# lelecaruso/NavierStokes_Project_NM4PDE

Measured on AMD Instinct MI355X. Metric: time-steps/sec (assemble_time_step + solve_time_step), 3D flow past a cylinder, P2/P1, Yosida, per-rank ILU(0), higher is better.
Workload: dtype f64

## Files before the change

navierstokes_project_nm4pde_amd/csrc/nsx_cg.hip:

```cpp
#include "nsx_grid.hpp"

namespace nsx {

constexpr int CG_THREADS = 256;
constexpr int CG_NW = CG_THREADS / 64, CG_NG = CG_THREADS / 16;
constexpr int CG_MAXB = 256;
constexpr int CG_MAX_WG = 1024;
constexpr int CG_NV = 3;
constexpr int CG_RING = 4;
constexpr size_t CG_REGION = (size_t)CG_RING * CG_NV * CG_MAX_WG + (size_t)CG_RING * CG_NV;
enum { S_CGP = 100 };

__device__ __forceinline__ double ld_agent(const double *p) { return __hip_atomic_load(p, __ATOMIC_RELAXED, __HIP_MEMORY_SCOPE_AGENT); }
__device__ __forceinline__ void st_agent(double *p, double v) { __hip_atomic_store(p, v, __ATOMIC_RELAXED, __HIP_MEMORY_SCOPE_AGENT); }

template <int W>
__device__ __forceinline__ double cg_group_sum(double v) {
  v += dpp_f64<0xB1>(v);
  v += dpp_f64<0x4E>(v);
  if (W >= 8) v += dpp_f64<0x141>(v);
  if (W >= 16) v += dpp_f64<0x140>(v);
  return v;
}

struct CgBox {
  unsigned long long *row, *row2, *total, *total2;
};
__device__ __forceinline__ CgBox cg_box_of(unsigned long long *box, int e) {
  CgBox b;
  b.row = box + (size_t)(e % CG_RING) * CG_NV * CG_MAX_WG;
  b.row2 = box + (size_t)((e + 2) % CG_RING) * CG_NV * CG_MAX_WG;
  b.total = box + (size_t)CG_RING * CG_NV * CG_MAX_WG + (size_t)(e % CG_RING) * CG_NV;
  b.total2 = box + (size_t)CG_RING * CG_NV * CG_MAX_WG + (size_t)((e + 2) % CG_RING) * CG_NV;
  return b;
}
__device__ __forceinline__ double cg_sum8(const double *w) {
  if (CG_NW == 4) return (w[0] + w[1]) + (w[2] + w[3]);
  return ((w[0] + w[1]) + (w[2] + w[3])) + ((w[4] + w[5]) + (w[6] + w[7]));
}

template <int NV>
__device__ __forceinline__ void cg_post(const double (&part)[NV], unsigned long long *box, int e, int nwg, double (*sh)[CG_NV * 8], int *s_err, bool drop = false) {
  const int wg = blockIdx.x, tid = threadIdx.x, wave = tid >> 6;
  const CgBox bx = cg_box_of(box, e);
  double *buf = sh[2 * (e & 1)], *buf0 = sh[2 * (e & 1) + 1];
  double ws[NV];
#pragma unroll
  for (int v = 0; v < NV; ++v) ws[v] = gx_wave_sum(part[v]);
  asm volatile("s_waitcnt vmcnt(0)" ::: "memory");
  if ((tid & 63) == 0) {
#pragma unroll
    for (int v = 0; v < NV; ++v) buf[v * 8 + wave] = ws[v];
  }
  __syncthreads();
  if (tid == 0) {
#pragma unroll
    for (int v = 0; v < NV; ++v)
      if (!drop) gx_post(bx.row + (size_t)v * CG_MAX_WG + wg, cg_sum8(buf + v * 8));
#pragma unroll
    for (int v = 0; v < CG_NV; ++v) gx_clear(bx.row2 + (size_t)v * CG_MAX_WG + wg);
  }
  if (wg == 0) {
    int lerr = 0;
    double a[NV];
#pragma unroll
    for (int v = 0; v < NV; ++v) a[v] = 0.0;
    for (int q = tid; q < nwg; q += CG_THREADS) {
      double m[NV];
      gx_wait_n<NV>(bx.row + q, CG_MAX_WG, m, &lerr);
#pragma unroll
      for (int v = 0; v < NV; ++v) a[v] += m[v];
    }
    if (lerr) *s_err = 1;
#pragma unroll
    for (int v = 0; v < NV; ++v) ws[v] = gx_wave_sum(a[v]);
    if ((tid & 63) == 0) {
#pragma unroll
      for (int v = 0; v < NV; ++v) buf0[v * 8 + wave] = ws[v];
    }
    __syncthreads();
    if (tid == 0 && !*s_err) {
#pragma unroll
      for (int v = 0; v < NV; ++v) gx_post(bx.total + v, cg_sum8(buf0 + v * 8));
    }
    if (tid < CG_NV) gx_clear(bx.total2 + tid);
  }
}
template <int NV>
__device__ __forceinline__ bool cg_collect(double (&tot)[NV], unsigned long long *box, int e, double *bc, int *s_err) {
  if (threadIdx.x == 0) {
    int lerr = 0;
    double m[NV];
    gx_wait_n<NV>(cg_box_of(box, e).total, 1, m, &lerr);
#pragma unroll
    for (int v = 0; v < NV; ++v) bc[v] = m[v];
    if (lerr) *s_err = 1;
  }
  __syncthreads();
#pragma unroll
  for (int v = 0; v < NV; ++v) tot[v] = bc[v];
  return *s_err == 0;
}
constexpr int CG_PF = 8;
constexpr int CG_MAX_UCOLS = 1024;
constexpr int CG_LPOOL = 6656;

__global__ void k_cg_pack(int64_t n_slots, const int32_t *__restrict__ src, const double *__restrict__ sv, double *__restrict__ out) {
  const int64_t i = (int64_t)blockIdx.x * blockDim.x + threadIdx.x;
  if (i < n_slots) out[i] = src[i] >= 0 ? sv[src[i]] : 0.0;
}

#define NSX_CG_LOAD(V, L, S0)                                   \
  _Pragma("unroll") for (int k = 0; k < CG_PF; ++k) {           \
    const int s_ = (S0) + k;                                    \
    const bool ok_ = s_ < s1;                                   \
    V[k] = ok_ ? sval[(size_t)s_ * 256 + tid] : 0.0;            \
    L[k] = ok_ ? (int)slidx[(size_t)s_ * 256 + tid] : 0;        \
  }
__device__ __forceinline__ void cg_spmv_prefetch(int s0, int s1, const double *__restrict__ sval, const uint16_t *__restrict__ slidx, int tid,
                                                 double (&va)[CG_PF], int (&la)[CG_PF]) {
  NSX_CG_LOAD(va, la, s0)
}
__device__ __forceinline__ void cg_block_spmv(int s0, int s1, const double *__restrict__ sval, const uint16_t *__restrict__ slidx,
                                              const int32_t *__restrict__ sinfo, const double *xst, double *hvs, int tid ,
                                              double (&va)[CG_PF], int (&la)[CG_PF]) {
  const int grp = tid >> 4, lane = tid & 15;
  double vb[CG_PF];
  int lb[CG_PF];
  double acc = 0.0;
#define NSX_CG_USE(V, L, S0)                                    \
  _Pragma("unroll") for (int k = 0; k < CG_PF; ++k) {           \
    const int s_ = (S0) + k;                                    \
    if (s_ < s1) {                                              \
      acc += V[k] * xst[L[k]];                                  \
      const int inf = sinfo[s_];                                \
      if (inf & 0x8000) {                                       \
        const double r_ = cg_group_sum<16>(acc);                \
        if (lane == 0) hvs[(inf & 0x7fff) * 16 + grp] = r_;     \
        acc = 0.0;                                              \
      }                                                         \
    }                                                           \
  }
  for (int sb = s0; sb < s1; sb += 2 * CG_PF) {
    NSX_CG_LOAD(vb, lb, sb + CG_PF)
    NSX_CG_USE(va, la, sb)
    NSX_CG_LOAD(va, la, sb + 2 * CG_PF)
    NSX_CG_USE(vb, lb, sb + CG_PF)
  }
#undef NSX_CG_USE
}
#undef NSX_CG_LOAD

template <int RPG, bool LRES>
__global__ __launch_bounds__(CG_THREADS) void k_cg_schur(const int32_t *__restrict__ bptr, const int32_t *__restrict__ u_ptr,
                                                  const int32_t *__restrict__ u_cols, const int32_t *__restrict__ s_ptr,
                                                  const double *__restrict__ sval, const uint16_t *__restrict__ slidx,
                                                  const int32_t *__restrict__ sinfo, const int64_t *__restrict__ dn_off,
                                                  const double *__restrict__ P, const double *__restrict__ b, double *x, double *D0, double *D1,
                                                  double *H, double rtol, int maxiter, unsigned long long *box, unsigned long long *box_other,
                                                  double *pub_vals, unsigned long long *pub_flag, unsigned long long seq, int *err_dev, int drop_wg,
                                                  const int32_t *__restrict__ a_rowptr, const double *__restrict__ a_val,
                                                  const uint16_t *__restrict__ a_lidx) {
  static_assert(!LRES || RPG > 0, "the LDS-resident operator needs the register-resident block inverses");
  constexpr int MAXB = RPG > 0 ? 16 * RPG : CG_MAXB;
  __shared__ double gs[MAXB], hs[MAXB], ds[MAXB], hvs[MAXB], xs[MAXB], xst[CG_MAX_UCOLS];
  __shared__ double sh[4][CG_NV * 8], bc[CG_NV];
  __shared__ int s_err;
  __shared__ double lval[LRES ? CG_LPOOL : 1];
  __shared__ uint16_t lidx[LRES ? CG_LPOOL : 2];
  __shared__ int lrow[LRES ? MAXB + 1 : 1];
  const int wg = blockIdx.x, tid = threadIdx.x, nwg = gridDim.x;
  if (tid == 0) s_err = 0;
  for (size_t q = (size_t)wg * CG_THREADS + tid; q < CG_REGION; q += (size_t)nwg * CG_THREADS) box_other[q] = GX_EMPTY;
  const int r0 = bptr[wg], nb = bptr[wg + 1] - r0;
  const int u0 = u_ptr[wg], nu = u_ptr[wg + 1] - u0;
  const int half = tid >> 8, ht = tid & 255;
  const int s0 = s_ptr[3 * wg + half], s1 = s_ptr[3 * wg + (CG_THREADS == 512 ? half + 1 : 2)];
  const double *Pb = P + dn_off[wg];
  const int grp = tid >> 4, lane = tid & 15;
  const bool own = tid < nb;
  int e = 0;
  constexpr int NU = CG_MAX_UCOLS / CG_THREADS;
  int ucol[NU];
#pragma unroll
  for (int k = 0; k < NU; ++k) ucol[k] = tid + CG_THREADS * k < nu ? u_cols[u0 + tid + CG_THREADS * k] : -1;
  if (tid < MAXB) gs[tid] = 0.0;

  double pa[8], pb[8];
  auto fetch = [&](int q, double(&pv)[8]) {
    const bool live = q < nb;
    const double *prow = Pb + (size_t)(live ? q : 0) * nb;
#pragma unroll
    for (int c = 0; c < 8; ++c) {
      const int j = lane + 16 * c;
      pv[c] = (live && j < nb) ? prow[j] : 0.0;
    }
  };
  constexpr bool PRES = RPG > 0;
  double pr[PRES ? RPG : 1][PRES ? RPG : 1];
  if constexpr (PRES) {
#pragma unroll
    for (int r = 0; r < RPG; ++r) {
      const int q = grp + CG_NG * r;
      const double *prow = Pb + (size_t)(q < nb ? q : 0) * nb;
#pragma unroll
      for (int c = 0; c < RPG; ++c) {
        const int j = lane + 16 * c;
        pr[r][c] = (q < nb && j < nb) ? prow[j] : 0.0;
      }
    }
  }
  auto prefetch_P = [&]() {
    if constexpr (!PRES) {
      if (nb <= 128) {
        fetch(grp, pa);
        fetch(grp + CG_NG, pb);
      }
    }
  };
  auto apply_P = [&]() {
    if constexpr (PRES) {
#pragma unroll
      for (int r = 0; r < RPG; ++r) {
        const int q = grp + CG_NG * r;
        if (q < nb) {
          double acc = 0.0;
#pragma unroll
          for (int c = 0; c < RPG; ++c) acc += pr[r][c] * gs[lane + 16 * c];
          acc = cg_group_sum<16>(acc);
          if (lane == 0) hs[q] = acc;
        }
      }
    } else if (nb <= 128) {
      auto use = [&](int q, const double(&pv)[8]) {
        if (q >= nb) return;
        double acc = 0.0;
#pragma unroll
        for (int c = 0; c < 8; ++c) acc += pv[c] * gs[lane + 16 * c];
        acc = cg_group_sum<16>(acc);
        if (lane == 0) hs[q] = acc;
      };
      for (int q = grp; q < nb; q += 2 * CG_NG) {
        use(q, pa);
        fetch(q + 2 * CG_NG, pa);
        use(q + CG_NG, pb);
        fetch(q + 3 * CG_NG, pb);
      }
    } else {
      for (int q = grp; q < nb; q += CG_NG) {
        const double *prow = Pb + (size_t)q * nb;
        double pv[16];
#pragma unroll
        for (int c = 0; c < 16; ++c) {
          const int j = lane + 16 * c;
          pv[c] = j < nb ? prow[j] : 0.0;
        }
        double acc = 0.0;
#pragma unroll
        for (int c = 0; c < 16; ++c) acc += pv[c] * gs[lane + 16 * c];
        acc = cg_group_sum<16>(acc);
        if (lane == 0) hs[q] = acc;
      }
    }
    __syncthreads();
    if (own) st_agent(H + r0 + tid, hs[tid]);
  };

  double va[LRES ? 1 : CG_PF];
  int la[LRES ? 1 : CG_PF];
  if constexpr (LRES) {
    const int p0 = a_rowptr[r0], nz = a_rowptr[r0 + nb] - p0;
    for (int q = tid; q < nz; q += CG_THREADS) {
      lval[q] = a_val[p0 + q];
      lidx[q] = a_lidx[p0 + q];
    }
    if (tid <= nb) lrow[tid] = a_rowptr[r0 + tid] - p0;
  }
  auto prefetch_A = [&]() {
    if constexpr (!LRES) cg_spmv_prefetch(s0, s1, sval, slidx, ht, va, la);
  };
  auto block_spmv = [&]() {
    if constexpr (LRES) {
#pragma unroll
      for (int r = 0; r < RPG; ++r) {
        const int q = grp + CG_NG * r;
        if (q < nb) {
          const int e1 = lrow[q + 1];
          double acc = 0.0;
          for (int e = lrow[q] + lane; e < e1; e += 16) acc += lval[e] * xst[lidx[e]];
          acc = cg_group_sum<16>(acc);
          if (lane == 0) hvs[q] = acc;
        }
      }
    } else {
      cg_block_spmv(s0, s1, sval, slidx, sinfo, xst, hvs, ht, va, la);
    }
  };

  double bi = 0.0;
  if (own) {
    xs[tid] = x[r0 + tid];
    bi = b[r0 + tid];
  }
#pragma unroll
  for (int k = 0; k < NU; ++k)
    if (ucol[k] >= 0) xst[tid + CG_THREADS * k] = x[ucol[k]];
  prefetch_A();
  __syncthreads();
  block_spmv();
  __syncthreads();
  prefetch_P();
  if (own) gs[tid] = hvs[tid] - bi;
  __syncthreads();
  apply_P();
  double tot3[3];
  {
    const double part[3] = {own ? gs[tid] * gs[tid] : 0.0, own ? bi * bi : 0.0, own ? gs[tid] * hs[tid] : 0.0};
    cg_post<3>(part, box, e, nwg, sh, &s_err, wg == drop_wg);
    prefetch_A();
    if (!cg_collect<3>(tot3, box, e++, bc, &s_err)) {
      if (tid == 0) __hip_atomic_store(err_dev, 1, __ATOMIC_RELAXED, __HIP_MEMORY_SCOPE_AGENT);
      if (wg == 0 && tid == 0) {
        __hip_atomic_store(pub_vals + 2, 3.0, __ATOMIC_RELAXED, __HIP_MEMORY_SCOPE_SYSTEM);
        asm volatile("s_waitcnt vmcnt(0)" ::: "memory");
        __hip_atomic_store(pub_flag, seq, __ATOMIC_RELAXED, __HIP_MEMORY_SCOPE_SYSTEM);
      }
      return;
    }
  }
  const double tol = rtol * sqrt(tot3[1]);
  double res = sqrt(tot3[0]), gh = tot3[2], beta = 0.0;
  int it = 0;
  int conv = res <= tol ? 1 : ((it >= maxiter || res != res) ? 2 : 0);
  bool dead = false;
  while (conv == 0) {
    ++it;
    const double *Dp = (it & 1) ? D0 : D1;
    double *Dc = (it & 1) ? D1 : D0;
#pragma unroll
    for (int k = 0; k < NU; ++k)
      if (ucol[k] >= 0) {
        const int j = ucol[k];
        xst[tid + CG_THREADS * k] = it == 1 ? -ld_agent(H + j) : __builtin_fma(beta, ld_agent(Dp + j), -ld_agent(H + j));
      }
    if (own) {
      const double dcur = it == 1 ? -hs[tid] : __builtin_fma(beta, ds[tid], -hs[tid]);
      ds[tid] = dcur;
      st_agent(Dc + r0 + tid, dcur);
    }
    __syncthreads();
    block_spmv();
    __syncthreads();
    double tot1[1];
    {
      const double part[1] = {own ? ds[tid] * hvs[tid] : 0.0};
      cg_post<1>(part, box, e, nwg, sh, &s_err);
      prefetch_P();
      if (!cg_collect<1>(tot1, box, e++, bc, &s_err)) {
        dead = true;
        break;
      }
    }
    const double alpha = gh / tot1[0];
    if (own) {
      xs[tid] += alpha * ds[tid];
      gs[tid] = gs[tid] + alpha * hvs[tid];
    }
    __syncthreads();
    apply_P();
    double tot2[2];
    {
      const double part[2] = {own ? gs[tid] * gs[tid] : 0.0, own ? gs[tid] * hs[tid] : 0.0};
      cg_post<2>(part, box, e, nwg, sh, &s_err);
      prefetch_A();
      if (!cg_collect<2>(tot2, box, e++, bc, &s_err)) {
        dead = true;
        break;
      }
    }
    res = sqrt(fabs(tot2[0]));
    conv = res <= tol ? 1 : ((it >= maxiter || res != res) ? 2 : 0);
    beta = tot2[1] / gh;
    gh = tot2[1];
  }
  if (dead && tid == 0) __hip_atomic_store(err_dev, 1, __ATOMIC_RELAXED, __HIP_MEMORY_SCOPE_AGENT);
  if (!dead && own) x[r0 + tid] = xs[tid];
  if (wg == 0 && tid == 0) {
    __hip_atomic_store(pub_vals + 0, (double)it, __ATOMIC_RELAXED, __HIP_MEMORY_SCOPE_SYSTEM);
    __hip_atomic_store(pub_vals + 1, res, __ATOMIC_RELAXED, __HIP_MEMORY_SCOPE_SYSTEM);
    __hip_atomic_store(pub_vals + 2, dead ? 3.0 : (conv == 1 ? 0.0 : 1.0), __ATOMIC_RELAXED, __HIP_MEMORY_SCOPE_SYSTEM);
    __hip_atomic_store(pub_vals + 3, tol, __ATOMIC_RELAXED, __HIP_MEMORY_SCOPE_SYSTEM);
    asm volatile("s_waitcnt vmcnt(0)" ::: "memory");
    __hip_atomic_store(pub_flag, seq, __ATOMIC_RELAXED, __HIP_MEMORY_SCOPE_SYSTEM);
  }
}

void build_cg_plan(nsx_handle *h) {
  CgPlan &pl = h->cgplan;
  pl.ok = false;
  const IluSchedule &s = h->schedS;
  if (!s.dense || s.max_rows > CG_MAXB) return;
  const Csr &g = h->gS.host;
  const std::vector<int32_t> &bptr = s.block_ptr_h;
  const int nb = s.n_blocks;
  std::vector<int32_t> u_ptr(nb + 1, 0), u_cols, s_ptr(3 * (size_t)nb + 1, 0), s_info, s_src, tmp;
  std::vector<uint16_t> s_lidx, a_lidx((size_t)g.nnz());
  pl.max_block_nnz = 0;
  for (int b = 0; b < nb; ++b) {
    const int r0 = bptr[b], r1 = bptr[b + 1], n = r1 - r0;
    tmp.assign(g.colind.begin() + g.rowptr[r0], g.colind.begin() + g.rowptr[r1]);
    std::sort(tmp.begin(), tmp.end());
    tmp.erase(std::unique(tmp.begin(), tmp.end()), tmp.end());
    if ((int)tmp.size() > CG_MAX_UCOLS) return;
    u_cols.insert(u_cols.end(), tmp.begin(), tmp.end());
    u_ptr[b + 1] = (int32_t)u_cols.size();
    pl.max_block_nnz = std::max(pl.max_block_nnz, g.rowptr[r1] - g.rowptr[r0]);
    for (int p = g.rowptr[r0]; p < g.rowptr[r1]; ++p) a_lidx[p] = (uint16_t)(std::lower_bound(tmp.begin(), tmp.end(), g.colind[p]) - tmp.begin());
    for (int half = 0; half < 2; ++half) {
      s_ptr[3 * (size_t)b + half] = (int32_t)s_info.size();
      for (int r = half; r * 16 < n; r += 2) {
        int maxlen = 0;
        for (int q = 16 * r; q < std::min(n, 16 * r + 16); ++q) maxlen = std::max(maxlen, g.rowptr[r0 + q + 1] - g.rowptr[r0 + q]);
        const int chunks = std::max(1, (maxlen + 15) / 16);
        for (int c = 0; c < chunks; ++c) {
          s_info.push_back(r | (c == chunks - 1 ? 0x8000 : 0));
          for (int t = 0; t < 256; ++t) {
            const int q = 16 * r + (t >> 4), e = 16 * c + (t & 15);
            int32_t src = -1;
            uint16_t li = 0;
            if (q < n && g.rowptr[r0 + q] + e < g.rowptr[r0 + q + 1]) {
              src = g.rowptr[r0 + q] + e;
              li = (uint16_t)(std::lower_bound(tmp.begin(), tmp.end(), g.colind[src]) - tmp.begin());
            }
            s_src.push_back(src);
            s_lidx.push_back(li);
          }
        }
      }
    }
    s_ptr[3 * (size_t)b + 2] = (int32_t)s_info.size();
  }
  pl.n_slots = (int64_t)s_src.size();
  pl.u_ptr.upload(u_ptr, h->stream);
  pl.u_cols.upload(u_cols, h->stream);
  pl.s_ptr.upload(s_ptr, h->stream);
  pl.s_info.upload(s_info, h->stream);
  pl.s_src.upload(s_src, h->stream);
  pl.s_lidx.upload(s_lidx, h->stream);
  pl.a_lidx.upload(a_lidx, h->stream);
  pl.s_val.alloc((size_t)pl.n_slots);
  pl.ok = true;
  pl.values_current = false;
  if (getenv("NSX_DEBUG"))
    fprintf(stderr, "[nsx] persistent Schur CG plan: %d blocks, %lld slabs (fill %.2f), unique columns per block avg %.0f\n", nb,
            (long long)s_info.size(), (double)g.nnz() / (double)std::max<int64_t>(1, pl.n_slots), (double)u_cols.size() / std::max(1, nb));
}

void cg_pack_values(nsx_handle *h) {
  CgPlan &pl = h->cgplan;
  if (!pl.ok) return;
  LaunchScope ls(h, "cg_pack", 20.0 * (double)pl.n_slots);
  hipLaunchKernelGGL(k_cg_pack, dim3(cdiv(pl.n_slots, 256)), dim3(256), 0, h->stream, pl.n_slots, pl.s_src.p, h->vSchur.p, pl.s_val.p);
  pl.values_current = true;
}

static void cg_setup(nsx_handle *h) {
  if (h->cg_box.p || h->cg_disabled) return;
  h->cg_max_wg = 0;
  if (getenv("NSX_CG_PERSISTENT") && atoi(getenv("NSX_CG_PERSISTENT")) == 0) {
    h->cg_disabled = true;
    return;
  }
  int cus = 0, per_cu = 0;
  HIP_CHECK(hipDeviceGetAttribute(&cus, hipDeviceAttributeMultiprocessorCount, h->prm.device));
  int per_cu_res[2] = {0, 0};
  HIP_CHECK(hipOccupancyMaxActiveBlocksPerMultiprocessor(&per_cu, k_cg_schur<0, false>, CG_THREADS, 0));
  HIP_CHECK(hipOccupancyMaxActiveBlocksPerMultiprocessor(&per_cu_res[0], k_cg_schur<6, false>, CG_THREADS, 0));
  HIP_CHECK(hipOccupancyMaxActiveBlocksPerMultiprocessor(&per_cu_res[1], k_cg_schur<8, false>, CG_THREADS, 0));
  h->cg_max_wg_res[0] = std::min(CG_MAX_WG, per_cu_res[0] * cus);
  h->cg_max_wg_res[1] = std::min(CG_MAX_WG, per_cu_res[1] * cus);
  int per_cu_lres[2] = {0, 0};
  HIP_CHECK(hipOccupancyMaxActiveBlocksPerMultiprocessor(&per_cu_lres[0], k_cg_schur<6, true>, CG_THREADS, 0));
  HIP_CHECK(hipOccupancyMaxActiveBlocksPerMultiprocessor(&per_cu_lres[1], k_cg_schur<8, true>, CG_THREADS, 0));
  h->cg_max_wg_lres[0] = std::min(CG_MAX_WG, per_cu_lres[0] * cus);
  h->cg_max_wg_lres[1] = std::min(CG_MAX_WG, per_cu_lres[1] * cus);
  h->cg_box.alloc(2 * CG_REGION + 2);
  HIP_CHECK(hipMemsetAsync(h->cg_box.p, 0xff, 2 * CG_REGION * sizeof(unsigned long long), h->stream));
  HIP_CHECK(hipMemsetAsync(h->cg_box.p + 2 * CG_REGION, 0, 2 * sizeof(unsigned long long), h->stream));
  h->cg_max_wg = std::min(CG_MAX_WG, per_cu * cus);
  if (getenv("NSX_DEBUG"))
    fprintf(stderr, "[nsx] persistent Schur CG: %d CUs x %d resident workgroups, grid <= %d (block inverses in registers: <= 96 rows x %d, <= 128 rows x %d; operator in LDS as well: x %d, x %d)\n", cus, per_cu,
            h->cg_max_wg, per_cu_res[0], per_cu_res[1], per_cu_lres[0], per_cu_lres[1]);
}

bool cg_schur_persistent(nsx_handle *h, double *x, const double *b, double rtol, int maxiter, int *steps, double *last, int *status) {
  const IluSchedule &s = h->schedS;
  const CgPlan &pl = h->cgplan;
  if (h->comm || !s.dense || s.max_rows > CG_MAXB || !pl.ok || !pl.values_current) return false;
  cg_setup(h);
  if (h->cg_max_wg == 0 || s.n_blocks > h->cg_max_wg) return false;
  const bool pres_ok = !(getenv("NSX_CG_PRES") && atoi(getenv("NSX_CG_PRES")) == 0);
  const int rpg = !pres_ok ? 0 : (s.max_rows <= 96 && s.n_blocks <= h->cg_max_wg_res[0]) ? 6 : (s.max_rows <= 128 && s.n_blocks <= h->cg_max_wg_res[1]) ? 8 : 0;
  const bool pres = rpg > 0;
  const bool lres_ok = !(getenv("NSX_CG_LRES") && atoi(getenv("NSX_CG_LRES")) == 0);
  const bool lres = lres_ok && pres && pl.max_block_nnz <= CG_LPOOL && s.n_blocks <= h->cg_max_wg_lres[rpg == 6 ? 0 : 1];
  const int n = h->n_p;
  if ((int)h->cg_vec.n < 3 * n) h->cg_vec.alloc((size_t)3 * n);
  double *D0 = h->cg_vec.p, *D1 = D0 + n, *H = D1 + n;
  const unsigned long long seq = ++h->pub_seq;
  unsigned long long *box = h->cg_box.p + (size_t)h->cg_parity * CG_REGION, *box_other = h->cg_box.p + (size_t)(1 - h->cg_parity) * CG_REGION;
  int *err_dev = (int *)(h->cg_box.p + 2 * CG_REGION);
  double *pub_vals = h->pub_dev + S_CGP;
  unsigned long long *pub_flag = (unsigned long long *)(h->pub_dev + N_SLOTS);
  ProfEntry *pe = nullptr;
  {
    LaunchScope ls(h, "cg_S", 0.0);
    pe = ls.e;
#define NSX_CG_GO(PRES_, LRES_)                                                                                                                       \
  hipLaunchKernelGGL((k_cg_schur<PRES_, LRES_>), dim3(s.n_blocks), dim3(CG_THREADS), 0, h->stream, s.block_ptr.p, pl.u_ptr.p, pl.u_cols.p, pl.s_ptr.p,  \
                     pl.s_val.p, pl.s_lidx.p, pl.s_info.p, s.dn_off.p, s.dn_P.p, b, x, D0, D1, H, rtol, maxiter, box, box_other, pub_vals, pub_flag, seq, \
                     err_dev, h->gx_drop_wg, h->gS.rowptr.p, h->vSchur.p, pl.a_lidx.p)
    if (rpg == 6 && lres) NSX_CG_GO(6, true); else if (rpg == 8 && lres) NSX_CG_GO(8, true);
    else if (rpg == 6) NSX_CG_GO(6, false); else if (rpg == 8) NSX_CG_GO(8, false); else NSX_CG_GO(0, false);
#undef NSX_CG_GO
    if (getenv("NSX_DEBUG") && (h->cg_resident != pres || h->cg_lds_resident != lres || !h->cg_variant_said)) {
      fprintf(stderr, "[nsx] Schur CG variant: block inverses in registers %d (rows per lane group %d), operator in LDS %d (largest block: %d entries)\n", (int)pres, rpg,
              (int)lres, (int)pl.max_block_nnz);
      h->cg_variant_said = true;
    }
    h->cg_resident = pres;
    h->cg_lds_resident = lres;
    h->cg_last_rpg = rpg;
    h->cg_last_lres = lres ? 1 : 0;
  }
  h->cg_parity ^= 1;
  h->cg_last_path = 2;
  wait_published(h, seq);
  const int st = (int)h->pub_host[S_CGP + 2];
  if (st == 3) {
    HIP_CHECK(hipStreamSynchronize(h->stream));
    HIP_CHECK(hipMemsetAsync(h->cg_box.p, 0xff, 2 * CG_REGION * sizeof(unsigned long long), h->stream));
    HIP_CHECK(hipMemsetAsync(h->cg_box.p + 2 * CG_REGION, 0, 2 * sizeof(unsigned long long), h->stream));
    h->cg_max_wg = 0;
    h->cg_disabled = true;
    h->n_persistent_fallbacks++;
    h->cg_last_rpg = h->cg_last_lres = 0;
    fprintf(stderr, "[nsx] warning: the persistent Schur CG timed out (grid not co-resident): this handle uses one launch per operation from now on\n");
    return false;
  }
  *steps = (int)h->pub_host[S_CGP];
  *last = h->pub_host[S_CGP + 1];
  *status = st;
  if (pe) pe->bytes += (lres ? 1.0 : (double)(*steps + 1)) * 10.0 * h->gS.nnz() + (double)(*steps + 1) * 48.0 * n + (pres ? 1.0 : (double)(*steps + 1)) * 8.0 * (double)s.dn_entries;
  return true;
}


constexpr int CGD_PARTS = 1024, CGD_FOLD_MAX = 8;
enum { CGD_DH = 0, CGD_P0 = CGD_PARTS, CGD_BB = 3 * CGD_PARTS, CGD_P1 = 4 * CGD_PARTS, CGD_TOTAL = 6 * CGD_PARTS };

__device__ __forceinline__ double cgd_sum(const double *__restrict__ p, double *sh) {
  double a = 0.0;
#pragma unroll
  for (int k = 0; k < CGD_PARTS / 256; ++k) a += p[threadIdx.x + 256 * k];
  return gx_block_sum(a, sh);
}
__device__ __forceinline__ void cgd_clear_tail(double *arrays, int n_arrays) {
  if (blockIdx.x != gridDim.x - 1 || (int)gridDim.x > CGD_PARTS) return;
  for (int a = 0; a < n_arrays; ++a)
    for (int q = (int)gridDim.x + (int)threadIdx.x; q < CGD_PARTS; q += CG_THREADS) arrays[(size_t)a * CGD_PARTS + q] = 0.0;
}
__global__ __launch_bounds__(256) void k_cgd_fold(int nblk, int grp, const double *__restrict__ raw, double *__restrict__ dst) {
  const int a = blockIdx.x >> 2, g = (blockIdx.x & 3) * 256 + threadIdx.x;
  const double *r = raw + (size_t)a * nblk;
  double s_ = 0.0;
  for (int k = 0; k < grp; ++k) {
    const int q = g * grp + k;
    if (q < nblk) s_ += r[q];
  }
  dst[(size_t)a * CGD_PARTS + g] = s_;
}
__device__ __forceinline__ void cgd_dense_apply(const double *__restrict__ Pb, int nb, const double *gs, double *hs, int tid) {
  const int grp = tid >> 4, lane = tid & 15;
  for (int q = grp; q < nb; q += CG_NG) {
    const double *prow = Pb + (size_t)q * nb;
    double pv[16];
#pragma unroll
    for (int c = 0; c < 16; ++c) {
      const int j = lane + 16 * c;
      pv[c] = j < nb ? prow[j] : 0.0;
    }
    double acc = 0.0;
#pragma unroll
    for (int c = 0; c < 16; ++c) acc += pv[c] * gs[lane + 16 * c];
    acc = cg_group_sum<16>(acc);
    if (lane == 0) hs[q] = acc;
  }
}

__global__ __launch_bounds__(CG_THREADS) void k_cgd_init(const int32_t *__restrict__ bptr, const int32_t *__restrict__ u_ptr, const int32_t *__restrict__ u_cols,
                                                   const int32_t *__restrict__ s_ptr, const double *__restrict__ sval, const uint16_t *__restrict__ slidx,
                                                   const int32_t *__restrict__ sinfo, const int64_t *__restrict__ dn_off, const double *__restrict__ P,
                                                   const double *__restrict__ b, const double *__restrict__ x, double *__restrict__ G, double *__restrict__ H,
                                                   double *__restrict__ out, int ostride) {
  __shared__ double gs[CG_MAXB], hs[CG_MAXB], hvs[CG_MAXB], xst[CG_MAX_UCOLS], sh[3][4];
  const int wg = blockIdx.x, tid = threadIdx.x;
  const int r0 = bptr[wg], nb = bptr[wg + 1] - r0, u0 = u_ptr[wg], nu = u_ptr[wg + 1] - u0;
  const int s0 = s_ptr[3 * wg], s1 = s_ptr[3 * wg + 2];
  const bool own = tid < nb;
  double va[CG_PF];
  int la[CG_PF];
  cg_spmv_prefetch(s0, s1, sval, slidx, tid, va, la);
  for (int k = tid; k < nu; k += CG_THREADS) xst[k] = x[u_cols[u0 + k]];
  gs[tid] = 0.0;
  const double bi = own ? b[r0 + tid] : 0.0;
  __syncthreads();
  cg_block_spmv(s0, s1, sval, slidx, sinfo, xst, hvs, tid, va, la);
  __syncthreads();
  if (own) {
    gs[tid] = hvs[tid] - bi;
    G[r0 + tid] = gs[tid];
  }
  __syncthreads();
  cgd_dense_apply(P + dn_off[wg], nb, gs, hs, tid);
  __syncthreads();
  if (own) H[r0 + tid] = hs[tid];
  const double gg = gx_block_sum(own ? gs[tid] * gs[tid] : 0.0, sh[0]);
  const double gh = gx_block_sum(own ? gs[tid] * hs[tid] : 0.0, sh[1]);
  const double bb = gx_block_sum(bi * bi, sh[2]);
  if (tid == 0) {
    out[wg] = gg;
    out[(size_t)ostride + wg] = gh;
    out[2 * (size_t)ostride + wg] = bb;
  }
  cgd_clear_tail(out, 3);
}

__global__ __launch_bounds__(256) void k_cgd_pack(int n_send, const int32_t *__restrict__ idx, int it, const double *__restrict__ parts, const double *__restrict__ H,
                                                  const double *__restrict__ Dp, double *__restrict__ buf) {
  __shared__ double sh[2][4];
  double beta = 0.0;
  if (it >= 2) {
    const double *cur = parts + (((it - 1) & 1) ? CGD_P1 : CGD_P0), *old = parts + (((it - 1) & 1) ? CGD_P0 : CGD_P1);
    beta = cgd_sum(cur + CGD_PARTS, sh[0]) / cgd_sum(old + CGD_PARTS, sh[1]);
  }
  const int k = blockIdx.x * 256 + threadIdx.x;
  if (k < n_send) {
    const int j = idx[k];
    buf[k] = it == 1 ? -H[j] : __builtin_fma(beta, Dp[j], -H[j]);
  }
}

__global__ __launch_bounds__(CG_THREADS) void k_cgd_A(const int32_t *__restrict__ bptr, const int32_t *__restrict__ u_ptr, const int32_t *__restrict__ u_cols,
                                                const int32_t *__restrict__ s_ptr, const double *__restrict__ sval, const uint16_t *__restrict__ slidx,
                                                const int32_t *__restrict__ sinfo, int n_own, int it, const double *__restrict__ parts, const double *__restrict__ H,
                                                const double *__restrict__ Dp, double *Dc, double *__restrict__ Hv, double *__restrict__ part_dh, double *pub_vals,
                                                unsigned long long *pub_flag, unsigned long long seq) {
  __shared__ double ds[CG_MAXB], hvs[CG_MAXB], xst[CG_MAX_UCOLS], sh[4][4];
  const int wg = blockIdx.x, tid = threadIdx.x;
  const int r0 = bptr[wg], nb = bptr[wg + 1] - r0, u0 = u_ptr[wg], nu = u_ptr[wg + 1] - u0;
  const int s0 = s_ptr[3 * wg], s1 = s_ptr[3 * wg + 2];
  const bool own = tid < nb;
  double va[CG_PF];
  int la[CG_PF];
  cg_spmv_prefetch(s0, s1, sval, slidx, tid, va, la);
  const double *cur = parts + (((it - 1) & 1) ? CGD_P1 : CGD_P0), *old = parts + (((it - 1) & 1) ? CGD_P0 : CGD_P1);
  const double gg = cgd_sum(cur, sh[0]), gh = cgd_sum(cur + CGD_PARTS, sh[1]);
  const double gh_old = it >= 2 ? cgd_sum(old + CGD_PARTS, sh[2]) : 1.0;
  const double beta = it >= 2 ? gh / gh_old : 0.0;
  if (wg == 0) {
    const double bb = it == 1 ? cgd_sum(parts + CGD_BB, sh[3]) : 0.0;
    if (tid == 0) {
      __hip_atomic_store(pub_vals + 0, gg, __ATOMIC_RELAXED, __HIP_MEMORY_SCOPE_SYSTEM);
      __hip_atomic_store(pub_vals + 1, bb, __ATOMIC_RELAXED, __HIP_MEMORY_SCOPE_SYSTEM);
      asm volatile("s_waitcnt vmcnt(0)" ::: "memory");
      __hip_atomic_store(pub_flag, seq, __ATOMIC_RELAXED, __HIP_MEMORY_SCOPE_SYSTEM);
    }
  }
  for (int k = tid; k < nu; k += CG_THREADS) {
    const int j = u_cols[u0 + k];
    xst[k] = j >= n_own ? Dc[j] : (it == 1 ? -H[j] : __builtin_fma(beta, Dp[j], -H[j]));
  }
  if (own) {
    const double dcur = it == 1 ? -H[r0 + tid] : __builtin_fma(beta, Dp[r0 + tid], -H[r0 + tid]);
    ds[tid] = dcur;
    Dc[r0 + tid] = dcur;
  }
  __syncthreads();
  cg_block_spmv(s0, s1, sval, slidx, sinfo, xst, hvs, tid, va, la);
  __syncthreads();
  if (own) Hv[r0 + tid] = hvs[tid];
  const double dh = gx_block_sum(own ? ds[tid] * hvs[tid] : 0.0, sh[3]);
  if (tid == 0) part_dh[wg] = dh;
  cgd_clear_tail(part_dh, 1);
}

__global__ __launch_bounds__(CG_THREADS) void k_cgd_B(const int32_t *__restrict__ bptr, const int64_t *__restrict__ dn_off, const double *__restrict__ P, int it,
                                                double *__restrict__ parts, double *__restrict__ x, double *__restrict__ G, double *__restrict__ H,
                                                const double *__restrict__ Dc, const double *__restrict__ Hv, double *__restrict__ out, int ostride) {
  __shared__ double gs[CG_MAXB], hs[CG_MAXB], sh[4][4];
  const int wg = blockIdx.x, tid = threadIdx.x;
  const int r0 = bptr[wg], nb = bptr[wg + 1] - r0;
  const bool own = tid < nb;
  const double *prev = parts + (((it - 1) & 1) ? CGD_P1 : CGD_P0);
  double *mine = out;
  const double dh = cgd_sum(parts + CGD_DH, sh[0]), gh = cgd_sum(prev + CGD_PARTS, sh[1]);
  const double alpha = gh / dh;
  gs[tid] = 0.0;
  __syncthreads();
  if (own) {
    x[r0 + tid] += alpha * Dc[r0 + tid];
    const double g = G[r0 + tid] + alpha * Hv[r0 + tid];
    gs[tid] = g;
    G[r0 + tid] = g;
  }
  __syncthreads();
  cgd_dense_apply(P + dn_off[wg], nb, gs, hs, tid);
  __syncthreads();
  if (own) H[r0 + tid] = hs[tid];
  const double gg = gx_block_sum(own ? gs[tid] * gs[tid] : 0.0, sh[2]);
  const double ghn = gx_block_sum(own ? gs[tid] * hs[tid] : 0.0, sh[3]);
  if (tid == 0) {
    mine[wg] = gg;
    mine[(size_t)ostride + wg] = ghn;
  }
  cgd_clear_tail(mine, 2);
}

bool cg_schur_fused(nsx_handle *h, double *x, const double *b, double rtol, int maxiter, int *steps, double *last, int *status) {
  const IluSchedule &s = h->schedS;
  const CgPlan &pl = h->cgplan;
  const bool wanted = !(getenv("NSX_CG_FUSED") && atoi(getenv("NSX_CG_FUSED")) == 0);
  if (!wanted) return false;
  if (h->cgd_agreed < 0)
    h->cgd_agreed = comm_agree_all(h, s.dense && s.max_rows <= CG_MAXB && pl.ok && s.n_blocks <= CGD_PARTS * CGD_FOLD_MAX && CG_THREADS == 256) ? 1 : 0;
  if (!h->cgd_agreed) return false;
  if (!pl.values_current) cg_pack_values(h);
  const int n = h->n_p, len = h->len_p, nblk = s.n_blocks;
  const bool fold = nblk > CGD_PARTS;
  const int fold_grp = cdiv(nblk, CGD_PARTS);
  if (fold && (int)h->cgd_raw.n < 3 * nblk) h->cgd_raw.alloc((size_t)3 * nblk);
  auto fold_into = [&](double *dst, int n_arrays) {
    if (fold) hipLaunchKernelGGL(k_cgd_fold, dim3(4 * n_arrays), dim3(256), 0, h->stream, nblk, fold_grp, h->cgd_raw.p, dst);
  };
  h->cg_last_path = 3;
  if ((int)h->cgd_vec.n < 3 * n + 2 * len) {
    h->cgd_vec.alloc((size_t)3 * n + 2 * len);
    h->cgd_vec.zero(h->stream);
  }
  if (!h->cgd_parts.p) {
    h->cgd_parts.alloc(CGD_TOTAL);
    h->cgd_parts.zero(h->stream);
  }
  double *G = h->cgd_vec.p, *H = G + n, *Hv = H + n, *D[2] = {Hv + n, Hv + n + len}, *parts = h->cgd_parts.p;
  double *pub_vals = h->pub_dev + S_CGP;
  unsigned long long *pub_flag = (unsigned long long *)(h->pub_dev + N_SLOTS);
  comm_halo_p(h, x);
  {
    LaunchScope ls(h, "cgd_init", 12.0 * h->gS.nnz() + 8.0 * (double)s.dn_entries + 40.0 * n);
    hipLaunchKernelGGL(k_cgd_init, dim3(nblk), dim3(CG_THREADS), 0, h->stream, s.block_ptr.p, pl.u_ptr.p, pl.u_cols.p, pl.s_ptr.p, pl.s_val.p, pl.s_lidx.p,
                       pl.s_info.p, s.dn_off.p, s.dn_P.p, b, x, G, H, fold ? h->cgd_raw.p : parts + CGD_P0, fold ? nblk : CGD_PARTS);
    fold_into(parts + CGD_P0, 3);
  }
  comm_allreduce_partials(h, parts + CGD_P0, 3 * CGD_PARTS);
  int it = 0, conv = 0;
  double tol = 0.0, res = 0.0;
  static const bool trace = getenv("NSX_TRACE") != nullptr;
  for (;;) {
    const int nx = it + 1;
    if (trace && (it < 3 || it % 200 == 0)) fprintf(stderr, "[nsx trace] rank %d: Schur CG iteration %d, residual %.3e, tolerance %.3e\n", h->rank, it, res, tol);
    double *Dp = D[(nx + 1) & 1], *Dc = D[nx & 1];
    if (h->dist && !h->haloP.nbr.empty()) {
      const std::function<void(hipStream_t, double *, const int32_t *, int)> packer = [&](hipStream_t st, double *buf, const int32_t *idx, int n_send) {
        if (n_send) hipLaunchKernelGGL(k_cgd_pack, dim3(cdiv(n_send, 256)), dim3(256), 0, st, n_send, idx, nx, parts, H, Dp, buf);
      };
      comm_halo_begin(h, h->haloP, Dc, 1, &packer);
      comm_halo_finish(h, h->haloP, Dc, 1);
    }
    const unsigned long long seq = ++h->pub_seq;
    {
      LaunchScope ls(h, "cgd_A", 10.0 * h->gS.nnz() + 40.0 * n);
      hipLaunchKernelGGL(k_cgd_A, dim3(nblk), dim3(CG_THREADS), 0, h->stream, s.block_ptr.p, pl.u_ptr.p, pl.u_cols.p, pl.s_ptr.p, pl.s_val.p, pl.s_lidx.p, pl.s_info.p,
                         n, nx, parts, H, Dp, Dc, Hv, fold ? h->cgd_raw.p : parts + CGD_DH, pub_vals, pub_flag, seq);
      fold_into(parts + CGD_DH, 1);
    }
    comm_allreduce_partials(h, parts + CGD_DH, CGD_PARTS);
    wait_published(h, seq);
    if (it == 0) tol = rtol * std::sqrt(h->pub_host[S_CGP + 1]);
    res = std::sqrt(std::fabs(h->pub_host[S_CGP]));
    conv = res <= tol ? 1 : ((it >= maxiter || res != res) ? 2 : 0);
    if (conv != 0) break;
    it = nx;
    {
      LaunchScope ls(h, "cgd_B", 8.0 * (double)s.dn_entries + 56.0 * n);
      double *mine = parts + ((it & 1) ? CGD_P1 : CGD_P0);
      hipLaunchKernelGGL(k_cgd_B, dim3(nblk), dim3(CG_THREADS), 0, h->stream, s.block_ptr.p, s.dn_off.p, s.dn_P.p, it, parts, x, G, H, Dc, Hv, fold ? h->cgd_raw.p : mine,
                         fold ? nblk : CGD_PARTS);
      fold_into(mine, 2);
    }
    comm_allreduce_partials(h, parts + ((it & 1) ? CGD_P1 : CGD_P0), 2 * CGD_PARTS);
  }
  *steps = it;
  *last = res;
  *status = conv == 1 ? 0 : 1;
  return true;
}

int cg_dirty_words(nsx_handle *h) {
  if (!h->cg_box.p) return 0;
  std::vector<unsigned long long> w(2 * CG_REGION);
  HIP_CHECK(hipStreamSynchronize(h->stream));
  HIP_CHECK(hipMemcpy(w.data(), h->cg_box.p, w.size() * sizeof(unsigned long long), hipMemcpyDeviceToHost));
  const size_t base = (size_t)h->cg_parity * CG_REGION;
  int dirty = 0;
  for (size_t q = 0; q < CG_REGION; ++q) dirty += w[base + q] != GX_EMPTY;
  return dirty;
}

}
```

Measured before the change: 14.45.

## Batch Schur CG prologue loads, unroll LDS SpMV, and add wave timestamp tracing

Reworks the persistent Schur CG kernel's prologue so the operator, row pointers, own x/b and ghost x values are all loaded into registers before any LDS stores. The goal is to overlap these global-memory latencies instead of serialising them. The LDS-resident SpMV now processes several rows at a time with fixed-depth unrolled gathers and FMAs, and the per-iteration ghost loads of H and D are batched ahead of use. It also adds an optional per-wave wall-clock trace, enabled by an environment variable, whose null-pointer check costs a little even when tracing is off. The extra register arrays raise register pressure.

```diff
diff --git a/navierstokes_project_nm4pde_amd/csrc/nsx_cg.hip b/navierstokes_project_nm4pde_amd/csrc/nsx_cg.hip
--- a/navierstokes_project_nm4pde_amd/csrc/nsx_cg.hip
+++ b/navierstokes_project_nm4pde_amd/csrc/nsx_cg.hip
@@ -104,6 +104,8 @@
 constexpr int CG_PF = 8;
 constexpr int CG_MAX_UCOLS = 1024;
 constexpr int CG_LPOOL = 6656;
+constexpr int CG_TRACE_ITS = 7, CG_TRACE_N = 64;
+static_assert(9 + 7 * CG_TRACE_ITS <= CG_TRACE_N, "stamps per wave");
 
 __global__ void k_cg_pack(int64_t n_slots, const int32_t *__restrict__ src, const double *__restrict__ sv, double *__restrict__ out) {
   const int64_t i = (int64_t)blockIdx.x * blockDim.x + threadIdx.x;
@@ -160,7 +162,7 @@
                                                   double *H, double rtol, int maxiter, unsigned long long *box, unsigned long long *box_other,
                                                   double *pub_vals, unsigned long long *pub_flag, unsigned long long seq, int *err_dev, int drop_wg,
                                                   const int32_t *__restrict__ a_rowptr, const double *__restrict__ a_val,
-                                                  const uint16_t *__restrict__ a_lidx) {
+                                                  const uint16_t *__restrict__ a_lidx, unsigned long long *trace = nullptr) {
   static_assert(!LRES || RPG > 0, "the LDS-resident operator needs the register-resident block inverses");
   constexpr int MAXB = RPG > 0 ? 16 * RPG : CG_MAXB;
   __shared__ double gs[MAXB], hs[MAXB], ds[MAXB], hvs[MAXB], xs[MAXB], xst[CG_MAX_UCOLS];
@@ -170,6 +172,14 @@
   __shared__ uint16_t lidx[LRES ? CG_LPOOL : 2];
   __shared__ int lrow[LRES ? MAXB + 1 : 1];
   const int wg = blockIdx.x, tid = threadIdx.x, nwg = gridDim.x;
+#define CG_STAMP(k)                                                                       \
+  do {                                                                                    \
+    if (trace && (tid & 63) == 0 && (k) < CG_TRACE_N) {                                   \
+      asm volatile("s_waitcnt vmcnt(0) lgkmcnt(0)" ::: "memory");                         \
+      trace[((size_t)wg * CG_NW + (tid >> 6)) * CG_TRACE_N + (k)] = wall_clock64();       \
+    }                                                                                     \
+  } while (0)
+  CG_STAMP(0);
   if (tid == 0) s_err = 0;
   for (size_t q = (size_t)wg * CG_THREADS + tid; q < CG_REGION; q += (size_t)nwg * CG_THREADS) box_other[q] = GX_EMPTY;
   const int r0 = bptr[wg], nb = bptr[wg + 1] - r0;
@@ -180,11 +190,20 @@
   const int grp = tid >> 4, lane = tid & 15;
   const bool own = tid < nb;
   int e = 0;
+  int p0 = 0, nz = 0;
+  if constexpr (LRES) {
+    p0 = a_rowptr[r0];
+    nz = a_rowptr[r0 + nb] - p0;
+  }
+  CG_STAMP(1);
   constexpr int NU = CG_MAX_UCOLS / CG_THREADS;
   int ucol[NU];
 #pragma unroll
-  for (int k = 0; k < NU; ++k) ucol[k] = tid + CG_THREADS * k < nu ? u_cols[u0 + tid + CG_THREADS * k] : -1;
-  if (tid < MAXB) gs[tid] = 0.0;
+  for (int k = 0; k < NU; ++k) {
+    const int c = tid + CG_THREADS * k;
+    const int v = u_cols[c < nu ? u0 + c : 0];
+    ucol[k] = c < nu ? v : -1;
+  }
 
   double pa[8], pb[8];
   auto fetch = [&](int q, double(&pv)[8]) {
@@ -268,28 +287,95 @@
 
   double va[LRES ? 1 : CG_PF];
   int la[LRES ? 1 : CG_PF];
+  constexpr int LB = CG_LPOOL / CG_THREADS / 2;
+  static_assert(2 * LB * CG_THREADS == CG_LPOOL, "two register sets hold the pool");
+  constexpr bool TWO_SETS = RPG <= 6;
+  double sva[LRES ? LB : 1], svb[LRES && TWO_SETS ? LB : 1];
+  int sca[LRES ? LB : 1], scb[LRES && TWO_SETS ? LB : 1], lr = 0;
+  const bool more = nz > LB * CG_THREADS;
+  auto stage_load = [&](int k0, double *sv, int *sc) {
+#pragma unroll
+    for (int k = 0; k < LB; ++k) {
+      const int q = tid + CG_THREADS * (k0 + k);
+      sv[k] = a_val[q < nz ? p0 + q : 0];
+      sc[k] = a_lidx[q < nz ? p0 + q : 0];
+    }
+  };
+  auto stage_store = [&](int k0, const double *sv, const int *sc) {
+#pragma unroll
+    for (int k = 0; k < LB; ++k) {
+      const int q = tid + CG_THREADS * (k0 + k);
+      if (q < nz) {
+        lval[q] = sv[k];
+        lidx[q] = (uint16_t)sc[k];
+      }
+    }
+  };
   if constexpr (LRES) {
-    const int p0 = a_rowptr[r0], nz = a_rowptr[r0 + nb] - p0;
-    for (int q = tid; q < nz; q += CG_THREADS) {
-      lval[q] = a_val[p0 + q];
-      lidx[q] = a_lidx[p0 + q];
-    }
-    if (tid <= nb) lrow[tid] = a_rowptr[r0 + tid] - p0;
-  }
+    lr = a_rowptr[r0 + (tid <= nb ? tid : 0)];
+    stage_load(0, sva, sca);
+    if constexpr (TWO_SETS)
+      if (more) stage_load(LB, svb, scb);
+  }
+  const double x_own = x[own ? r0 + tid : 0], b_own = b[own ? r0 + tid : 0];
+  double xg[NU];
+#pragma unroll
+  for (int k = 0; k < NU; ++k) xg[k] = x[ucol[k] >= 0 ? ucol[k] : 0];
+  CG_STAMP(2);
+  if (tid < MAXB) gs[tid] = 0.0;
+  if constexpr (LRES) {
+    stage_store(0, sva, sca);
+    if (more) {
+      if constexpr (TWO_SETS) {
+        stage_store(LB, svb, scb);
+      } else {
+        stage_load(LB, sva, sca);
+        stage_store(LB, sva, sca);
+      }
+    }
+    if (tid <= nb) lrow[tid] = lr - p0;
+  }
+  CG_STAMP(3);
   auto prefetch_A = [&]() {
     if constexpr (!LRES) cg_spmv_prefetch(s0, s1, sval, slidx, ht, va, la);
   };
   auto block_spmv = [&]() {
     if constexpr (LRES) {
-#pragma unroll
-      for (int r = 0; r < RPG; ++r) {
-        const int q = grp + CG_NG * r;
-        if (q < nb) {
-          const int e1 = lrow[q + 1];
+      constexpr int RI = RPG <= 6 ? 3 : 2, LT = RPG <= 6 ? 6 : 4;
+#pragma unroll
+      for (int rb = 0; rb < RPG; rb += RI) {
+        int e0[RI], e1[RI], ci[RI][LT];
+        double av[RI][LT], xv[RI][LT];
+#pragma unroll
+        for (int i = 0; i < RI; ++i) {
+          const int q = grp + CG_NG * (rb + i);
+          e0[i] = lrow[q < nb ? q : 0] + lane;
+          e1[i] = lrow[q < nb ? q + 1 : 0];
+        }
+#pragma unroll
+        for (int i = 0; i < RI; ++i) {
+          if (grp + CG_NG * (rb + i) >= nb) e1[i] = 0;
+#pragma unroll
+          for (int t = 0; t < LT; ++t) {
+            const int en = e0[i] + 16 * t, es = en < e1[i] ? en : 0;
+            ci[i][t] = lidx[es];
+            av[i][t] = lval[es];
+          }
+        }
+#pragma unroll
+        for (int i = 0; i < RI; ++i)
+#pragma unroll
+          for (int t = 0; t < LT; ++t) xv[i][t] = xst[ci[i][t]];
+#pragma unroll
+        for (int i = 0; i < RI; ++i) {
+          const int q = grp + CG_NG * (rb + i);
           double acc = 0.0;
-          for (int e = lrow[q] + lane; e < e1; e += 16) acc += lval[e] * xst[lidx[e]];
+#pragma unroll
+          for (int t = 0; t < LT; ++t)
+            acc = e0[i] + 16 * t < e1[i] ? __builtin_fma(av[i][t], xv[i][t], acc) : acc;
+          for (int en = e0[i] + 16 * LT; en < e1[i]; en += 16) acc = __builtin_fma(lval[en], xst[lidx[en]], acc);
           acc = cg_group_sum<16>(acc);
-          if (lane == 0) hvs[q] = acc;
+          if (lane == 0 && q < nb) hvs[q] = acc;
         }
       }
     } else {
@@ -297,26 +383,27 @@
     }
   };
 
-  double bi = 0.0;
-  if (own) {
-    xs[tid] = x[r0 + tid];
-    bi = b[r0 + tid];
-  }
+  const double bi = own ? b_own : 0.0;
+  if (own) xs[tid] = x_own;
 #pragma unroll
   for (int k = 0; k < NU; ++k)
-    if (ucol[k] >= 0) xst[tid + CG_THREADS * k] = x[ucol[k]];
+    if (ucol[k] >= 0) xst[tid + CG_THREADS * k] = xg[k];
   prefetch_A();
   __syncthreads();
+  CG_STAMP(4);
   block_spmv();
   __syncthreads();
+  CG_STAMP(5);
   prefetch_P();
   if (own) gs[tid] = hvs[tid] - bi;
   __syncthreads();
   apply_P();
+  CG_STAMP(6);
   double tot3[3];
   {
     const double part[3] = {own ? gs[tid] * gs[tid] : 0.0, own ? bi * bi : 0.0, own ? gs[tid] * hs[tid] : 0.0};
     cg_post<3>(part, box, e, nwg, sh, &s_err, wg == drop_wg);
+    CG_STAMP(7);
     prefetch_A();
     if (!cg_collect<3>(tot3, box, e++, bc, &s_err)) {
       if (tid == 0) __hip_atomic_store(err_dev, 1, __ATOMIC_RELAXED, __HIP_MEMORY_SCOPE_AGENT);
@@ -328,6 +415,7 @@
       return;
     }
   }
+  CG_STAMP(8);
   const double tol = rtol * sqrt(tot3[1]);
   double res = sqrt(tot3[0]), gh = tot3[2], beta = 0.0;
   int it = 0;
@@ -337,30 +425,49 @@
     ++it;
     const double *Dp = (it & 1) ? D0 : D1;
     double *Dc = (it & 1) ? D1 : D0;
-#pragma unroll
-    for (int k = 0; k < NU; ++k)
-      if (ucol[k] >= 0) {
-        const int j = ucol[k];
-        xst[tid + CG_THREADS * k] = it == 1 ? -ld_agent(H + j) : __builtin_fma(beta, ld_agent(Dp + j), -ld_agent(H + j));
-      }
+    {
+      double hn[NU], dn[NU];
+      if (it == 1) {
+#pragma unroll
+        for (int k = 0; k < NU; ++k) hn[k] = ld_agent(H + (ucol[k] >= 0 ? ucol[k] : 0));
+#pragma unroll
+        for (int k = 0; k < NU; ++k)
+          if (ucol[k] >= 0) xst[tid + CG_THREADS * k] = -hn[k];
+      } else {
+#pragma unroll
+        for (int k = 0; k < NU; ++k) {
+          const int j = ucol[k] >= 0 ? ucol[k] : 0;
+          dn[k] = ld_agent(Dp + j);
+          hn[k] = ld_agent(H + j);
+        }
+#pragma unroll
+        for (int k = 0; k < NU; ++k)
+          if (ucol[k] >= 0) xst[tid + CG_THREADS * k] = __builtin_fma(beta, dn[k], -hn[k]);
+      }
+    }
     if (own) {
       const double dcur = it == 1 ? -hs[tid] : __builtin_fma(beta, ds[tid], -hs[tid]);
       ds[tid] = dcur;
       st_agent(Dc + r0 + tid, dcur);
     }
     __syncthreads();
+    const int ts = 9 + 7 * (it - 1);
+    CG_STAMP(ts);
     block_spmv();
     __syncthreads();
+    CG_STAMP(ts + 1);
     double tot1[1];
     {
       const double part[1] = {own ? ds[tid] * hvs[tid] : 0.0};
       cg_post<1>(part, box, e, nwg, sh, &s_err);
+      CG_STAMP(ts + 2);
       prefetch_P();
       if (!cg_collect<1>(tot1, box, e++, bc, &s_err)) {
         dead = true;
         break;
       }
     }
+    CG_STAMP(ts + 3);
     const double alpha = gh / tot1[0];
     if (own) {
       xs[tid] += alpha * ds[tid];
@@ -368,16 +475,19 @@
     }
     __syncthreads();
     apply_P();
+    CG_STAMP(ts + 4);
     double tot2[2];
     {
       const double part[2] = {own ? gs[tid] * gs[tid] : 0.0, own ? gs[tid] * hs[tid] : 0.0};
       cg_post<2>(part, box, e, nwg, sh, &s_err);
+      CG_STAMP(ts + 5);
       prefetch_A();
       if (!cg_collect<2>(tot2, box, e++, bc, &s_err)) {
         dead = true;
         break;
       }
     }
+    CG_STAMP(ts + 6);
     res = sqrt(fabs(tot2[0]));
     conv = res <= tol ? 1 : ((it >= maxiter || res != res) ? 2 : 0);
     beta = tot2[1] / gh;
@@ -393,6 +503,7 @@
     asm volatile("s_waitcnt vmcnt(0)" ::: "memory");
     __hip_atomic_store(pub_flag, seq, __ATOMIC_RELAXED, __HIP_MEMORY_SCOPE_SYSTEM);
   }
+#undef CG_STAMP
 }
 
 void build_cg_plan(nsx_handle *h) {
@@ -493,6 +604,33 @@
             h->cg_max_wg, per_cu_res[0], per_cu_res[1], per_cu_lres[0], per_cu_lres[1]);
 }
 
+static void cg_trace_dump(nsx_handle *h, const DevBuf<unsigned long long> &buf, const char *path, int launch, int nwg, int rpg, bool lres, int steps) {
+  std::vector<unsigned long long> tr((size_t)nwg * CG_NW * CG_TRACE_N);
+  buf.download(tr.data(), tr.size(), h->stream);
+  FILE *f = fopen(path, "w");
+  if (!f) return;
+  fprintf(f, "# k_cg_schur<%d,%s> launch %d: %d workgroups, %d iterations; per wave: workgroup wave rows ucols entries, then %d stamps in ticks of 10 ns relative to the grid's first stamp (-1: not reached)\n"
+             "# 0 start, 1 descriptors read, 2 P_b in registers, 3 operator in LDS, 4 first gather, 5 first product, 6 first apply_P, 7 exchange 0 posted, 8 collected; then per iteration:\n"
+             "# gather done, product done, exchange 1 posted, collected, update and apply_P done, exchange 2 posted, collected\n",
+          rpg, lres ? "true" : "false", launch, nwg, steps, CG_TRACE_N);
+  unsigned long long t0 = ~0ull;
+  for (size_t q = 0; q < tr.size(); q += CG_TRACE_N)
+    if (tr[q]) t0 = std::min(t0, tr[q]);
+  const std::vector<int32_t> &bp = h->schedS.block_ptr_h, &rp = h->gS.host.rowptr;
+  std::vector<int32_t> up((size_t)nwg + 1);
+  h->cgplan.u_ptr.download(up.data(), up.size(), h->stream);
+  for (int b = 0; b < nwg; ++b)
+    for (int w = 0; w < CG_NW; ++w) {
+      fprintf(f, "%d %d %d %d %d", b, w, bp[b + 1] - bp[b], up[b + 1] - up[b], rp[bp[b + 1]] - rp[bp[b]]);
+      for (int k = 0; k < CG_TRACE_N; ++k) {
+        const unsigned long long v = tr[((size_t)b * CG_NW + w) * CG_TRACE_N + k];
+        fprintf(f, " %lld", v ? (long long)(v - t0) : -1ll);
+      }
+      fprintf(f, "\n");
+    }
+  fclose(f);
+}
+
 bool cg_schur_persistent(nsx_handle *h, double *x, const double *b, double rtol, int maxiter, int *steps, double *last, int *status) {
   const IluSchedule &s = h->schedS;
   const CgPlan &pl = h->cgplan;
@@ -513,13 +651,21 @@
   double *pub_vals = h->pub_dev + S_CGP;
   unsigned long long *pub_flag = (unsigned long long *)(h->pub_dev + N_SLOTS);
   ProfEntry *pe = nullptr;
+  static int n_launches = 0;
+  DevBuf<unsigned long long> trace_buf;
+  const char *trace_path = getenv("NSX_CG_TRACE");
+  const bool traced = trace_path && ++n_launches == (getenv("NSX_CG_TRACE_CALL") ? atoi(getenv("NSX_CG_TRACE_CALL")) : 100);
+  if (traced) {
+    trace_buf.alloc((size_t)s.n_blocks * CG_NW * CG_TRACE_N);
+    trace_buf.zero(h->stream);
+  }
   {
     LaunchScope ls(h, "cg_S", 0.0);
     pe = ls.e;
 #define NSX_CG_GO(PRES_, LRES_)                                                                                                                       \
   hipLaunchKernelGGL((k_cg_schur<PRES_, LRES_>), dim3(s.n_blocks), dim3(CG_THREADS), 0, h->stream, s.block_ptr.p, pl.u_ptr.p, pl.u_cols.p, pl.s_ptr.p,  \
                      pl.s_val.p, pl.s_lidx.p, pl.s_info.p, s.dn_off.p, s.dn_P.p, b, x, D0, D1, H, rtol, maxiter, box, box_other, pub_vals, pub_flag, seq, \
-                     err_dev, h->gx_drop_wg, h->gS.rowptr.p, h->vSchur.p, pl.a_lidx.p)
+                     err_dev, h->gx_drop_wg, h->gS.rowptr.p, h->vSchur.p, pl.a_lidx.p, trace_buf.p)
     if (rpg == 6 && lres) NSX_CG_GO(6, true); else if (rpg == 8 && lres) NSX_CG_GO(8, true);
     else if (rpg == 6) NSX_CG_GO(6, false); else if (rpg == 8) NSX_CG_GO(8, false); else NSX_CG_GO(0, false);
 #undef NSX_CG_GO
@@ -551,6 +697,7 @@
   *steps = (int)h->pub_host[S_CGP];
   *last = h->pub_host[S_CGP + 1];
   *status = st;
+  if (traced) cg_trace_dump(h, trace_buf, trace_path, n_launches, s.n_blocks, rpg, lres, *steps);
   if (pe) pe->bytes += (lres ? 1.0 : (double)(*steps + 1)) * 10.0 * h->gS.nnz() + (double)(*steps + 1) * 48.0 * n + (pres ? 1.0 : (double)(*steps + 1)) * 8.0 * (double)s.dn_entries;
   return true;
 }
```

Result: no change. 14.54, median of 6 (+0.6%).
